# SUTD-MDQS/QILaplace.jl

Hardware: AMD Instinct MI355X
Metric: MPO×MPS site-contractions/sec + max |coeff err|, n=24 χ_s=64 χ_c=128 (higher is better)
Workload: dtype f64; 1 GPU; zt_n24_chi64_D128; sites=48, mps_bonds_max=64, mpo_bonds_max=128, parallelism=replicas x1 (one signal per GPU), ranks_reported_by_collective_backend=1

## Files before the change

### qilaplace.jl_amd/csrc/qil_linalg.hip

```cpp
#include <algorithm>
#include <chrono>
#include <cmath>
#include <cstring>
#include <numeric>
#include <utility>

#include "qil_internal.h"
#include "qil_launch.h"
#include "qil_device_utils.h"

namespace {

using namespace qil_dev;

constexpr int GK = 16;
#ifndef QIL_GEMM_GAUSS
#define QIL_GEMM_GAUSS 1
#endif
#ifndef QIL_GEMM_PAD
#define QIL_GEMM_PAD 2
#endif
constexpr int GPAD = QIL_GEMM_PAD;
typedef double d4 __attribute__((ext_vector_type(4)));

__device__ __forceinline__ void put_plane(double* S0, double* S1, int off, double v) {
    S0[off] = v;
    (void)S1;
}
__device__ __forceinline__ void put_plane(double* S0, double* S1, int off, c64 v) {
    S0[off] = v.re;
    S1[off] = v.im;
}
__device__ __forceinline__ double maybe_conj(double v, int) { return v; }
__device__ __forceinline__ c64 maybe_conj(c64 v, int cj) { return cj ? c64{v.re, -v.im} : v; }

template <class T, int BM, int BN, int WM, int WN, bool PIPE, bool ARC, bool BKC, int GKT = GK, int DEEP = 0>
__device__ __forceinline__ void gemm_mfma_body(const uint3 blockIdx, const uint3 gridDim, long long m, long long n, long long k_total,
                                                 const T* __restrict__ A, long long a_rs, long long a_ks, int conjA,
                                                 const T* __restrict__ B, long long b_ks, long long b_cs, int conjB,
                                                 T* __restrict__ C, long long ldc, long long kchunk,
                                                 long long cstride, int tiles_m, int tiles_n, int col_fastest,
                                                 long long a_bs, long long b_bs, long long c_bs,
                                                 const int* __restrict__ cmap, int cmap_blk,
                                                 const uint8_t* __restrict__ b_sel, long long b_sel_step,
                                                 long long b_sel_stride, int subtract) {
    constexpr bool CX = sizeof(T) == 16;
    constexpr int NP = CX ? 2 : 1;
    constexpr int LA = BM + GPAD, LB = BN + GPAD;
    constexpr int NBUF = PIPE ? 2 : 1;
    constexpr int TM = WM / 16, TN = WN / 16;
    constexpr int EA = BM * GKT / 256, EB = BN * GKT / 256;
    static_assert((BM / WM) * (BN / WN) == 4, "4 waves per workgroup");
    extern __shared__ __attribute__((aligned(16))) char gemm_smem[];
    double* As = reinterpret_cast<double*>(gemm_smem);
    double* Bs = As + NBUF * NP * GKT * LA;
    const int tid = threadIdx.x;
    const int lane = tid & 63, wave = tid >> 6;
    const int wr = (wave % (BM / WM)) * WM, wc = (wave / (BM / WM)) * WN;
    const int l15 = lane & 15, l4 = lane >> 4;
    int tile = blockIdx.x;
    if (col_fastest & 2) tile = (tile % 8) * (tiles_m * tiles_n / 8) + tile / 8;
    int tm, tn;
    if (col_fastest & 1) {
        tn = tile % tiles_n;
        tm = tile / tiles_n;
    } else {
        tm = tile % tiles_m;
        tn = tile / tiles_m;
    }
    const long long row0 = (long long)tm * BM, col0 = (long long)tn * BN;
    const long long kbeg = (long long)blockIdx.z * kchunk;
    const long long kend = min(k_total, kbeg + kchunk);
    A += (long long)blockIdx.y * a_bs;
    B += (long long)blockIdx.y * b_bs;
    if (b_sel) B += (long long)b_sel[(long long)blockIdx.y * b_sel_step] * b_sel_stride;
    C += (long long)blockIdx.z * cstride + (long long)blockIdx.y * c_bs;
    if (cmap) cmap += (long long)blockIdx.y * (n / cmap_blk);

    d4 rr[TM][TN], ii[CX ? TM : 1][CX ? TN : 1], ri[CX ? TM : 1][CX ? TN : 1];
#pragma unroll
    for (int a = 0; a < TM; ++a)
#pragma unroll
        for (int b = 0; b < TN; ++b) {
            rr[a][b] = d4{0, 0, 0, 0};
            if (CX) {
                ii[a][b] = d4{0, 0, 0, 0};
                ri[a][b] = d4{0, 0, 0, 0};
            }
        }
    constexpr bool a_rows_contig = ARC, b_k_contig = BKC;
    T ra[EA], rb[EB];
    const T* pa[EA];
    const T* pb[EB];
    int ka[EA], kb[EB], sa[EA], sb[EB];
#pragma unroll
    for (int e = 0; e < EA; ++e) {
        const int idx = tid + 256 * e;
        const int i = a_rows_contig ? idx % BM : idx / GKT;
        const int kk = a_rows_contig ? idx / BM : idx % GKT;
        const long long gr = row0 + i;
        ka[e] = kk;
        sa[e] = kk * LA + i;
        pa[e] = A + min(gr, m - 1) * a_rs + (kbeg + kk) * a_ks;
    }
#pragma unroll
    for (int e = 0; e < EB; ++e) {
        const int idx = tid + 256 * e;
        const int kk = b_k_contig ? idx % GKT : idx / BN;
        const int j = b_k_contig ? idx / GKT : idx % BN;
        const long long gc = col0 + j;
        kb[e] = kk;
        sb[e] = kk * LB + j;
        pb[e] = B + (kbeg + kk) * b_ks + min(gc, n - 1) * b_cs;
    }
    const long long a_step = (long long)GKT * a_ks, b_step = (long long)GKT * b_ks;
    auto load_tile_into = [&](T(&ra)[EA], T(&rb)[EB], long long k0) {
        if (k0 + GKT <= kend) {
#pragma unroll
            for (int e = 0; e < EA; ++e) {
                ra[e] = *pa[e];
                pa[e] += a_step;
            }
#pragma unroll
            for (int e = 0; e < EB; ++e) {
                rb[e] = *pb[e];
                pb[e] += b_step;
            }
        } else {
#pragma unroll
            for (int e = 0; e < EA; ++e) ra[e] = *((k0 + ka[e] < kend) ? pa[e] : A);
#pragma unroll
            for (int e = 0; e < EB; ++e) rb[e] = *((k0 + kb[e] < kend) ? pb[e] : B);
        }
    };
    auto load_tile = [&](long long k0) { load_tile_into(ra, rb, k0); };
    auto store_tile_from = [&](const T(&ra)[EA], const T(&rb)[EB], int buf, long long k0) {
        double* a0 = As + (buf * NP) * GKT * LA;
        double* b0 = Bs + (buf * NP) * GKT * LB;
        if (k0 + GKT <= kend) {
#pragma unroll
            for (int e = 0; e < EA; ++e) put_plane(a0, a0 + GKT * LA, sa[e], maybe_conj(ra[e], conjA));
#pragma unroll
            for (int e = 0; e < EB; ++e) put_plane(b0, b0 + GKT * LB, sb[e], maybe_conj(rb[e], conjB));
        } else {
#pragma unroll
            for (int e = 0; e < EA; ++e)
                put_plane(a0, a0 + GKT * LA, sa[e], (k0 + ka[e] < kend) ? maybe_conj(ra[e], conjA) : T{});
#pragma unroll
            for (int e = 0; e < EB; ++e)
                put_plane(b0, b0 + GKT * LB, sb[e], (k0 + kb[e] < kend) ? maybe_conj(rb[e], conjB) : T{});
        }
    };
    auto store_tile = [&](int buf, long long k0) { store_tile_from(ra, rb, buf, k0); };
    auto mfma_tile = [&](int buf) {
        const double* a0 = As + (buf * NP) * GKT * LA;
        const double* b0 = Bs + (buf * NP) * GKT * LB;
#pragma unroll
        for (int kk = 0; kk < GKT; kk += 4) {
            double are[TM], aim[TM], bre[TN], bim[TN];
#pragma unroll
            for (int t = 0; t < TM; ++t) {
                are[t] = a0[(kk + l4) * LA + wr + 16 * t + l15];
                if (CX) aim[t] = a0[GKT * LA + (kk + l4) * LA + wr + 16 * t + l15];
            }
#pragma unroll
            for (int t = 0; t < TN; ++t) {
                bre[t] = b0[(kk + l4) * LB + wc + 16 * t + l15];
                if (CX) bim[t] = b0[GKT * LB + (kk + l4) * LB + wc + 16 * t + l15];
            }
            if constexpr (CX && QIL_GEMM_GAUSS) {
                double asum[TM], bsum[TN], bdif[TN];
#pragma unroll
                for (int t = 0; t < TM; ++t) asum[t] = are[t] + aim[t];
#pragma unroll
                for (int t = 0; t < TN; ++t) {
                    bsum[t] = bre[t] + bim[t];
                    bdif[t] = bim[t] - bre[t];
                }
#pragma unroll
                for (int ti = 0; ti < TM; ++ti)
#pragma unroll
                    for (int tj = 0; tj < TN; ++tj) {
                        rr[ti][tj] = __builtin_amdgcn_mfma_f64_16x16x4f64(bre[tj], asum[ti], rr[ti][tj], 0, 0, 0);
                        ii[ti][tj] = __builtin_amdgcn_mfma_f64_16x16x4f64(bsum[tj], aim[ti], ii[ti][tj], 0, 0, 0);
                        ri[ti][tj] = __builtin_amdgcn_mfma_f64_16x16x4f64(bdif[tj], are[ti], ri[ti][tj], 0, 0, 0);
                    }
            } else {
#pragma unroll
                for (int ti = 0; ti < TM; ++ti)
#pragma unroll
                    for (int tj = 0; tj < TN; ++tj) {
                        rr[ti][tj] = __builtin_amdgcn_mfma_f64_16x16x4f64(bre[tj], are[ti], rr[ti][tj], 0, 0, 0);
                        if constexpr (CX) {
                            ii[ti][tj] = __builtin_amdgcn_mfma_f64_16x16x4f64(bim[tj], aim[ti], ii[ti][tj], 0, 0, 0);
                            ri[ti][tj] = __builtin_amdgcn_mfma_f64_16x16x4f64(bim[tj], are[ti], ri[ti][tj], 0, 0, 0);
                            ri[ti][tj] = __builtin_amdgcn_mfma_f64_16x16x4f64(bre[tj], aim[ti], ri[ti][tj], 0, 0, 0);
                        }
                    }
            }
        }
    };
    if constexpr (PIPE && DEEP) {
        T ra1[EA], rb1[EB];
        if (kbeg < kend) load_tile_into(ra, rb, kbeg);
        if (kbeg + GKT < kend) load_tile_into(ra1, rb1, kbeg + GKT);
        for (long long k0 = kbeg; k0 < kend; k0 += 2 * GKT) {
            store_tile_from(ra, rb, 0, k0);
            __syncthreads();
            if (k0 + 2 * GKT < kend) load_tile_into(ra, rb, k0 + 2 * GKT);
            mfma_tile(0);
            if (k0 + GKT >= kend) break;
            store_tile_from(ra1, rb1, 1, k0 + GKT);
            __syncthreads();
            if (k0 + 3 * GKT < kend) load_tile_into(ra1, rb1, k0 + 3 * GKT);
            mfma_tile(1);
        }
    } else {
        int buf = 0;
        if (PIPE && kbeg < kend) load_tile(kbeg);
        for (long long k0 = kbeg; k0 < kend; k0 += GKT) {
            if (!PIPE) {
                if (k0 > kbeg) __syncthreads();
                load_tile(k0);
            }
            store_tile(buf, k0);
            __syncthreads();
            if (PIPE && k0 + GKT < kend) load_tile(k0 + GKT);
            mfma_tile(buf);
            if (PIPE) buf ^= 1;
        }
    }
#pragma unroll
    for (int ti = 0; ti < TM; ++ti)
#pragma unroll
        for (int tj = 0; tj < TN; ++tj)
#pragma unroll
            for (int r = 0; r < 4; ++r) {
                const long long gr = row0 + wr + 16 * ti + l15;
                const long long gc = col0 + wc + 16 * tj + l4 + 4 * r;
                if (gr < m && gc < n) {
                    const long long oc = cmap ? (long long)cmap[gc / cmap_blk] * cmap_blk + gc % cmap_blk : gc;
                    double* cp = reinterpret_cast<double*>(C + gr + ldc * oc);
                    if (subtract) {
                        if (CX) {
                            cp[0] -= rr[ti][tj][r] - ii[ti][tj][r];
                            cp[1] -= QIL_GEMM_GAUSS ? rr[ti][tj][r] + ri[ti][tj][r] : ri[ti][tj][r];
                        } else {
                            cp[0] -= rr[ti][tj][r];
                        }
                    } else if (CX) {
                        cp[0] = rr[ti][tj][r] - ii[ti][tj][r];
                        cp[1] = QIL_GEMM_GAUSS ? rr[ti][tj][r] + ri[ti][tj][r] : ri[ti][tj][r];
                    } else {
                        cp[0] = rr[ti][tj][r];
                    }
                }
            }
}
template <class T, int BM, int BN, int WM, int WN, bool PIPE, bool ARC, bool BKC, int GKT = GK, int DEEP = 0>
struct gemm_mfma_k {
    static constexpr int NT = 256, MINW = (DEEP ? 1 : (BM * BN <= 128 * 128 ? 2 : 1));
    template <class... QA>
    static __device__ __forceinline__ void run(const uint3 b, const uint3 g, QA... a) {
        gemm_mfma_body<T, BM, BN, WM, WN, PIPE, ARC, BKC, GKT, DEEP>(b, g, a...);
    }
};

template <class T>
__device__ __forceinline__ void splitk_reduce_body(const uint3 blockIdx, const uint3 gridDim, const T* __restrict__ W, long long cstride, int splits, long long m, long long n,
                              T* __restrict__ C, long long ldc, int subtract) {
    for (long long t = blockIdx.x * (long long)blockDim.x + threadIdx.x; t < m * n;
         t += (long long)gridDim.x * blockDim.x) {
        T acc = W[t];
        for (int z = 1; z < splits; ++z) acc = add_t(acc, W[t + z * cstride]);
        T* cp = C + (t % m) + ldc * (t / m);
        *cp = subtract ? sub_t(*cp, acc) : acc;
    }
}
template <class T>
struct splitk_reduce_k {
    static constexpr int NT = 1024, MINW = 1;
    template <class... QA>
    static __device__ __forceinline__ void run(const uint3 b, const uint3 g, QA... a) {
        splitk_reduce_body<T>(b, g, a...);
    }
};

struct gemm_batch {
    int count = 1;
    long long a_bs = 0, b_bs = 0, c_bs = 0;
    const int* cmap = nullptr;
    int cmap_blk = 1;
    const uint8_t* b_sel = nullptr;
    long long b_sel_step = 0, b_sel_stride = 0;
    int subtract = 0;
    int skinny_m = 0;
};

struct gemm_shape {
    int bm, bn, wm, wn, gkt, deep;
};
enum { GS_32x64_DEEP, GS_48x64_DEEP, GS_32x32, GS_64x64, GS_64x144, GS_128x128, GS_128x64, GS_COUNT };
constexpr gemm_shape GEMM_SHAPES[GS_COUNT] = {
    {32, 64, 16, 32, GK, 1}, {48, 64, 48, 16, GK, 1}, {32, 32, 16, 16, 32, 0}, {64, 64, 32, 32, GK, 0},
    {64, 144, 16, 144, GK, 0}, {128, 128, 64, 64, GK, 0}, {128, 64, 64, 32, GK, 0}};

int gemm_pick_shape(bool cx, long long m, long long n, long long count, int skinny_m) {
    if (skinny_m && m <= 32 && n >= 128) return GS_32x64_DEEP;
    if (skinny_m && m <= 48 && n >= 128) return GS_48x64_DEEP;
    constexpr long long small_tiles = 64;
    if (((m + 63) / 64) * ((n + 63) / 64) * count <= small_tiles && m >= 32 && n >= 32) return GS_32x32;
    if (cx) return GS_64x64;
    if (m >= 256 && n > 96 && n <= 144) return GS_64x144;
    {
        const long long t128 = ((m + 127) / 128) * ((n + 127) / 128);
        const bool fills = (double)m * (double)n >= 0.85 * 16384.0 * (double)t128;
        if (t128 * count >= 512 && fills) return GS_128x128;
    }
    {
        constexpr long long min_tiles = 128;
        const long long t = ((m + 127) / 128) * ((n + 63) / 64) * count;
        if (m >= 256 && t >= min_tiles) return GS_128x64;
    }
    return GS_64x64;
}

int gemm_plan(bool cx, int opA, int opB, long long m, long long n, long long k, long long lda, long long ldb, long long ldc,
              long long count, long long c_bs, bool has_cmap, int skinny_m, qil_gemm_plan_info* p) {
    const int si = gemm_pick_shape(cx, m, n, count, skinny_m);
    const gemm_shape& s = GEMM_SHAPES[si];
    p->bm = s.bm, p->bn = s.bn, p->wm = s.wm, p->wn = s.wn, p->gkt = s.gkt, p->deep = s.deep;
    const bool at = opA == 1 || opA == 2, bt = opB == 1 || opB == 2;
    p->arc = (at ? lda : 1) == 1;
    p->bkc = (bt ? ldb : 1) == 1;
    const long long tiles_m = (m + s.bm - 1) / s.bm, tiles_n = (n + s.bn - 1) / s.bn;
    const long long tiles = tiles_m * tiles_n;
    p->tiles_m = tiles_m, p->tiles_n = tiles_n;
    const bool can_split = count == 1 || (ldc == m && c_bs == m * n && !has_cmap);
    p->can_split = can_split;
    int splits = 1, rule = 0;
    static const long long split_min_k = 1024;
    if (can_split && tiles * count < 128 && (k >= split_min_k || (k >= 512 && tiles * count <= 8))) {
        splits = (int)std::min<long long>(std::min<long long>(k / 256, 512 / (tiles * count)), 64);
        rule = 1;
    }
    if (can_split && tiles * count <= 4 && k >= 128) {
        const int s2 = (int)std::min<long long>(k / 64, 32);
        if (s2 > splits) splits = s2, rule = 2;
    }
    if (splits < 2 && can_split && tiles * count >= 128 && tiles * count <= 384 && k >= 4096) {
        splits = (int)std::min<long long>(4, (767 / (tiles * count)));
        rule = 3;
    }
    if (splits < 2) splits = 1, rule = 0;
    long long kchunk = k;
    if (splits > 1) {
        kchunk = (((k + splits - 1) / splits) + s.gkt - 1) / s.gkt * s.gkt;
        splits = (int)((k + kchunk - 1) / kchunk);
    }
    p->splits = splits, p->split_rule = rule, p->kchunk = kchunk;
    p->col_fastest = tiles_n <= 8 ? 1 : 0;
    p->xcd = tiles >= 64 && tiles % 8 == 0;
    return si;
}

template <class T, int SI>
int gemm_launch(qil_context* ctx, const qil_gemm_plan_info& p, long long m, long long n, long long k, const T* A, long long a_rs,
                long long a_ks, int conjA, const T* B, long long b_ks, long long b_cs, int conjB, T* C,
                long long ldc, const gemm_batch& bt) {
    constexpr gemm_shape S = GEMM_SHAPES[SI];
    constexpr int BM = S.bm, BN = S.bn, WM = S.wm, WN = S.wn, GKT = S.gkt, DEEP = S.deep;
    constexpr bool PIPE = true;
    constexpr int NP = sizeof(T) == 16 ? 2 : 1;
    constexpr size_t lds = (size_t)(PIPE ? 2 : 1) * NP * GKT * ((BM + GPAD) + (BN + GPAD)) * sizeof(double);
    const long long tiles = p.tiles_m * p.tiles_n;
    const int splits = p.splits;
    long long cstride = 0, c_bs = bt.c_bs;
    T* Cout = C;
    long long ldo = ldc;
    void* wsp = nullptr;
    if (splits > 1) {
        cstride = m * n * bt.count;
        c_bs = m * n;
        QIL_TRY(qil_ctx_alloc(ctx, (size_t)(cstride * splits) * sizeof(T), &wsp));
        Cout = static_cast<T*>(wsp);
        ldo = m;
    }
    const int order = p.col_fastest | (p.xcd ? 2 : 0);
#define QIL_GEMM_K(ARCv, BKCv)                                                                                               \
    QIL_TRY((qil_klaunch<gemm_mfma_k<T, BM, BN, WM, WN, PIPE, ARCv, BKCv, GKT, DEEP>>(                                                      \
        ctx, dim3((unsigned)tiles, (unsigned)bt.count, (unsigned)splits), dim3(256), lds, m, n, k, A, a_rs, a_ks, conjA, B, b_ks, \
        b_cs, conjB, Cout, ldo, (long long)p.kchunk, cstride, (int)p.tiles_m, (int)p.tiles_n, order, bt.a_bs, bt.b_bs, c_bs, bt.cmap,  \
        bt.cmap_blk, bt.b_sel, bt.b_sel_step, bt.b_sel_stride, splits > 1 ? 0 : bt.subtract)))
    if (p.arc && p.bkc) QIL_GEMM_K(true, true);
    else if (p.arc) QIL_GEMM_K(true, false);
    else if (p.bkc) QIL_GEMM_K(false, true);
    else QIL_GEMM_K(false, false);
#undef QIL_GEMM_K
    if (splits > 1) {
        QIL_TRY((qil_klaunch<splitk_reduce_k<T>>(ctx, dim3((unsigned)std::min<long long>((cstride + 255) / 256, 2048)), dim3(256), 0, (const T*)Cout, cstride, splits, m, n * bt.count, C, ldc, bt.subtract)));
        QIL_HIP(hipGetLastError());
        qil_ctx_free(ctx, wsp);
    }
    return QIL_OK;
}

template <class T>
int gemm_dispatch(qil_context* ctx, int opA, int opB, long long m, long long n, long long k, const T* A,
                  long long lda, const T* B, long long ldb, T* C, long long ldc,
                  const gemm_batch& batch = gemm_batch{}) {
    if (m == 0 || n == 0) return QIL_OK;
    QIL_REQUIRE(opA >= 0 && opA <= 3 && opB >= 0 && opB <= 3, QIL_EINVAL_ARG, "gemm: bad op codes %d, %d", opA, opB);
    const bool at = opA == 1 || opA == 2, bt = opB == 1 || opB == 2;
    const long long a_rs = at ? lda : 1, a_ks = at ? 1 : lda;
    const long long b_ks = bt ? ldb : 1, b_cs = bt ? 1 : ldb;
    const int cA = (opA == 2 || opA == 3) ? 1 : 0, cB = (opB == 2 || opB == 3) ? 1 : 0;
    constexpr bool CX = sizeof(T) == 16;
    qil_gemm_plan_info p;
    const int si = gemm_plan(CX, opA, opB, m, n, k, lda, ldb, ldc, batch.count, batch.c_bs, batch.cmap != nullptr, batch.skinny_m, &p);
#define QIL_GEMM_GO(SI) \
    case SI: return gemm_launch<T, SI>(ctx, p, m, n, k, A, a_rs, a_ks, cA, B, b_ks, b_cs, cB, C, ldc, batch)
    switch (si) {
        QIL_GEMM_GO(GS_32x64_DEEP);
        QIL_GEMM_GO(GS_48x64_DEEP);
        QIL_GEMM_GO(GS_32x32);
        QIL_GEMM_GO(GS_64x64);
    }
    if constexpr (!CX) {
        switch (si) {
            QIL_GEMM_GO(GS_64x144);
            QIL_GEMM_GO(GS_128x128);
            QIL_GEMM_GO(GS_128x64);
        }
    }
#undef QIL_GEMM_GO
    return qil_fail(QIL_EINVAL_ARG, "gemm: no kernel for tile shape %d", si);
}

template <class T>
__device__ __forceinline__ void jacobi_round_body(const uint3 blockIdx, const uint3 gridDim, T* __restrict__ A, long long lda, long long m,
                                                    T* __restrict__ V, long long ldv, int vrows, int n,
                                                    int npad, int round, double tol,
                                                    int* __restrict__ rotated,
                                                    const double* __restrict__ negligible) {
    __shared__ double red[16];
    const int i = blockIdx.x;
    int p, q;
    if (i == 0) {
        p = npad - 1;
        q = round;
    } else {
        p = (round + i) % (npad - 1);
        q = (round + npad - 1 - i) % (npad - 1);
    }
    if (p >= n || q >= n) return;
    if (p > q) {
        const int t = p;
        p = q;
        q = t;
    }
    T* ap = A + lda * p;
    T* aq = A + lda * q;
    double v[4] = {0, 0, 0, 0};
    for (long long r = threadIdx.x; r < m; r += 256) {
        const T x = ap[r], y = aq[r];
        v[0] += abs2_t(x);
        v[1] += abs2_t(y);
        dot_parts(x, y, v[2], v[3]);
    }
    block_sum<4>(v, red);
    if (negligible) {
        const double ng = *negligible;
        if (v[0] < ng || v[1] < ng) return;
    }
    double c, s, pr, pi;
    bool big;
    if (!jacobi_rotation<sizeof(T) == 16>(v[0], v[1], v[2], v[3], tol, c, s, pr, pi, big)) return;
    if (threadIdx.x == 0) {
        rotated[0] = 1;
        if (big) rotated[1] = 1;
    }
    for (long long r = threadIdx.x; r < m; r += 256) {
        T x = ap[r], y = aq[r];
        rotate_pair(x, y, c, s, pr, pi);
        ap[r] = x;
        aq[r] = y;
    }
    T* vp = V + ldv * p;
    T* vq = V + ldv * q;
    for (int r = threadIdx.x; r < vrows; r += 256) {
        T x = vp[r], y = vq[r];
        rotate_pair(x, y, c, s, pr, pi);
        vp[r] = x;
        vq[r] = y;
    }
}
template <class T>
struct jacobi_round_k {
    static constexpr int NT = 256, MINW = 1;
    template <class... QA>
    static __device__ __forceinline__ void run(const uint3 b, const uint3 g, QA... a) {
        jacobi_round_body<T>(b, g, a...);
    }
};


template <class T, int KM>
__device__ __forceinline__ int block_pair_rotate(T* __restrict__ ap, T* __restrict__ aq, int m, T* __restrict__ vp,
                                                 T* __restrict__ vq, int vrows, int lane, double tol, double ng) {
    double al = 0, be = 0, gr = 0, gi = 0;
    constexpr int KA = KM > 0 ? KM : 1;
    T xs[KA], ys[KA];
    if (KM > 0) {
#pragma unroll
        for (int k = 0; k < KA; ++k) {
            const int r = lane + 64 * k;
            xs[k] = r < m ? ap[r] : T{};
            ys[k] = r < m ? aq[r] : T{};
        }
#pragma unroll
        for (int k = 0; k < KA; ++k) {
            al += abs2_t(xs[k]);
            be += abs2_t(ys[k]);
            dot_parts(xs[k], ys[k], gr, gi);
        }
    } else {
        for (int r = lane; r < m; r += 64) {
            const T x = ap[r], y = aq[r];
            al += abs2_t(x);
            be += abs2_t(y);
            dot_parts(x, y, gr, gi);
        }
    }
    al = wave_sum(al);
    be = wave_sum(be);
    gr = wave_sum(gr);
    if (sizeof(T) == 16) gi = wave_sum(gi);
    double c, sn, pr, pi;
    bool big;
    if (al < ng || be < ng || !jacobi_rotation<sizeof(T) == 16>(al, be, gr, gi, tol, c, sn, pr, pi, big)) return 0;
    if (KM > 0) {
        T us[KA], ws[KA];
#pragma unroll
        for (int k = 0; k < KA; ++k) {
            const int r = lane + 64 * k;
            us[k] = r < vrows ? vp[r] : T{};
            ws[k] = r < vrows ? vq[r] : T{};
        }
#pragma unroll
        for (int k = 0; k < KA; ++k) {
            const int r = lane + 64 * k;
            rotate_pair(xs[k], ys[k], c, sn, pr, pi);
            if (r < m) {
                ap[r] = xs[k];
                aq[r] = ys[k];
            }
        }
#pragma unroll
        for (int k = 0; k < KA; ++k) {
            const int r = lane + 64 * k;
            rotate_pair(us[k], ws[k], c, sn, pr, pi);
            if (r < vrows) {
                vp[r] = us[k];
                vq[r] = ws[k];
// ... 3856 lines not shown
```

Baseline: 3904 site-contractions/s.

## Generalize deep GEMM pipeline to NS register sets with unchecked steady-state loads

Replaces the fixed two-stage register prefetch in the deep MFMA GEMM path with a configurable ring of NS register tile sets. The steady-state loop uses unchecked global loads with pointer increments, sched barriers and compiler fences, falling back to a bounds-checked loop for the tail. It also raises the deep kernel's minimum waves-per-EU hint from 1 to 2. This aims to hide global-memory latency and cut per-tile bounds checks, but it adds register pressure that the higher occupancy hint may push into spills.

Result: no change. 3949 site-contractions/s, median of 4 (+1.2%).

```diff
diff --git a/qilaplace.jl_amd/csrc/qil_linalg.hip b/qilaplace.jl_amd/csrc/qil_linalg.hip
--- a/qilaplace.jl_amd/csrc/qil_linalg.hip
+++ b/qilaplace.jl_amd/csrc/qil_linalg.hip
@@ -21,6 +21,16 @@
 #define QIL_GEMM_PAD 2
 #endif
 constexpr int GPAD = QIL_GEMM_PAD;
+#ifndef QIL_DEEP_NS32
+#define QIL_DEEP_NS32 2
+#endif
+#ifndef QIL_DEEP_NS48
+#define QIL_DEEP_NS48 2
+#endif
+#ifndef QIL_DEEP_MINW
+#define QIL_DEEP_MINW 2
+#endif
+constexpr int gemm_deep_sets(int bm) { return bm <= 32 ? QIL_DEEP_NS32 : QIL_DEEP_NS48; }
 typedef double d4 __attribute__((ext_vector_type(4)));
 
 __device__ __forceinline__ void put_plane(double* S0, double* S1, int off, double v) {
@@ -30,6 +40,12 @@
 __device__ __forceinline__ void put_plane(double* S0, double* S1, int off, c64 v) {
     S0[off] = v.re;
     S1[off] = v.im;
+}
+typedef double d2g __attribute__((ext_vector_type(2), aligned(8)));
+__device__ __forceinline__ double load_global(const double* p) { return *(const __attribute__((address_space(1))) double*)p; }
+__device__ __forceinline__ c64 load_global(const c64* p) {
+    const d2g v = *(const __attribute__((address_space(1))) d2g*)p;
+    return c64{v.x, v.y};
 }
 __device__ __forceinline__ double maybe_conj(double v, int) { return v; }
 __device__ __forceinline__ c64 maybe_conj(c64 v, int cj) { return cj ? c64{v.re, -v.im} : v; }
@@ -201,19 +217,72 @@
         }
     };
     if constexpr (PIPE && DEEP) {
-        T ra1[EA], rb1[EB];
-        if (kbeg < kend) load_tile_into(ra, rb, kbeg);
-        if (kbeg + GKT < kend) load_tile_into(ra1, rb1, kbeg + GKT);
-        for (long long k0 = kbeg; k0 < kend; k0 += 2 * GKT) {
-            store_tile_from(ra, rb, 0, k0);
-            __syncthreads();
-            if (k0 + 2 * GKT < kend) load_tile_into(ra, rb, k0 + 2 * GKT);
-            mfma_tile(0);
-            if (k0 + GKT >= kend) break;
-            store_tile_from(ra1, rb1, 1, k0 + GKT);
-            __syncthreads();
-            if (k0 + 3 * GKT < kend) load_tile_into(ra1, rb1, k0 + 3 * GKT);
-            mfma_tile(1);
+        constexpr int NS = gemm_deep_sets(BM);
+        constexpr int U = NS % 2 ? 2 * NS : NS;
+        T rsa[NS][EA], rsb[NS][EB];
+        auto load_full = [&](T(&qa)[EA], T(&qb)[EB]) {
+#pragma unroll
+            for (int e = 0; e < EA; ++e) {
+                qa[e] = load_global(pa[e]);
+                pa[e] += a_step;
+                asm volatile("" : "+v"(pa[e]));
+            }
+#pragma unroll
+            for (int e = 0; e < EB; ++e) {
+                qb[e] = load_global(pb[e]);
+                pb[e] += b_step;
+                asm volatile("" : "+v"(pb[e]));
+            }
+        };
+        auto load_any = [&](T(&qa)[EA], T(&qb)[EB], long long k0) {
+            if (k0 + GKT <= kend) {
+                load_full(qa, qb);
+            } else {
+#pragma unroll
+                for (int e = 0; e < EA; ++e) qa[e] = load_global((k0 + ka[e] < kend) ? pa[e] : A);
+#pragma unroll
+                for (int e = 0; e < EB; ++e) qb[e] = load_global((k0 + kb[e] < kend) ? pb[e] : B);
+            }
+        };
+        auto store_full = [&](const T(&qa)[EA], const T(&qb)[EB], int buf) {
+            double* a0 = As + (buf * NP) * GKT * LA;
+            double* b0 = Bs + (buf * NP) * GKT * LB;
+#pragma unroll
+            for (int e = 0; e < EA; ++e) put_plane(a0, a0 + GKT * LA, sa[e], maybe_conj(qa[e], conjA));
+#pragma unroll
+            for (int e = 0; e < EB; ++e) put_plane(b0, b0 + GKT * LB, sb[e], maybe_conj(qb[e], conjB));
+        };
+        const long long klen = kend - kbeg;
+        const long long nfull = klen / GKT, ntile = (klen + GKT - 1) / GKT;
+        long long t = 0;
+        if (nfull >= U + NS) {
+#pragma unroll
+            for (int s = 0; s < NS; ++s) load_full(rsa[s], rsb[s]);
+            do {
+#pragma unroll
+                for (int s = 0; s < U; ++s) {
+                    __builtin_amdgcn_sched_barrier(0);
+                    store_full(rsa[s % NS], rsb[s % NS], s & 1);
+                    __syncthreads();
+                    load_full(rsa[s % NS], rsb[s % NS]);
+                    mfma_tile(s & 1);
+                }
+                t += U;
+            } while (t + U + NS <= nfull);
+        } else {
+#pragma unroll
+            for (int s = 0; s < NS; ++s)
+                if (s < ntile) load_any(rsa[s], rsb[s], kbeg + s * GKT);
+        }
+        for (; t < ntile; t += U) {
+#pragma unroll
+            for (int s = 0; s < U; ++s) {
+                if (t + s >= ntile) break;
+                store_tile_from(rsa[s % NS], rsb[s % NS], s & 1, kbeg + (t + s) * GKT);
+                __syncthreads();
+                if (t + s + NS < ntile) load_any(rsa[s % NS], rsb[s % NS], kbeg + (t + s + NS) * GKT);
+                mfma_tile(s & 1);
+            }
         }
     } else {
         int buf = 0;
@@ -259,7 +328,7 @@
 }
 template <class T, int BM, int BN, int WM, int WN, bool PIPE, bool ARC, bool BKC, int GKT = GK, int DEEP = 0>
 struct gemm_mfma_k {
-    static constexpr int NT = 256, MINW = (DEEP ? 1 : (BM * BN <= 128 * 128 ? 2 : 1));
+    static constexpr int NT = 256, MINW = (DEEP ? QIL_DEEP_MINW : (BM * BN <= 128 * 128 ? 2 : 1));
     template <class... QA>
     static __device__ __forceinline__ void run(const uint3 b, const uint3 g, QA... a) {
         gemm_mfma_body<T, BM, BN, WM, WN, PIPE, ARC, BKC, GKT, DEEP>(b, g, a...);
```
